# bcgsc/RNA-Bloom

Measured on AMD Instinct MI355X. Metric: k-mers/sec hashed+inserted into Bloom dBG (k=25, 50M 150bp reads), higher is better.
Workload: dtype u64

## Files before the change

rna-bloom_amd/csrc/rb_batch.hip:

```cpp
#include <math.h>
#include <stdlib.h>
#include <string.h>

#include <algorithm>
#include <vector>

#include "rb_internal.hpp"
#include "rb_kernels.hpp"

using namespace rb;

namespace {

constexpr int TPB = 256;
inline unsigned blocks_for(int64_t n, int tpb = TPB) { return (unsigned)((n + tpb - 1) / tpb); }

template <bool PIECE>
__global__ void k_encode_ascii_t(const uint8_t *__restrict__ seq, const uint8_t *__restrict__ qual,
                                 const int64_t *__restrict__ off, const uint32_t *__restrict__ woff,
                                 int64_t n_reads, int64_t n_words, int min_q,
                                 uint64_t *__restrict__ codes, uint32_t *__restrict__ valid,
                                 uint32_t *__restrict__ word_read, uint32_t *__restrict__ rnz,
                                 int64_t r_first, int64_t seq_base) {
    int64_t w = (int64_t)blockIdx.x * blockDim.x + threadIdx.x;
// ... 580 lines not shown
                      uint64_t *__restrict__ keys, uint32_t *__restrict__ vals, const uint32_t *__restrict__ keepmask,
                      const ulonglong2 *__restrict__ wstate) {
    constexpr uint32_t SLAB = RB_EMIT_SLAB, BW = RB_SPARSE_WORDS;
    __shared__ uint64_t s_key[SLAB + SLAB / 32 + 1];
    __shared__ uint32_t s_val[SLAB + SLAB / 32 + 1];
    __shared__ uint64_t s_tf[25], s_tr[25];
    __shared__ uint16_t s_list[BW];
    const uint32_t uk = (uint32_t)k, lane = threadIdx.x;
    const int64_t blk0 = (int64_t)blockIdx.x * BW;
    const int64_t blk_end = (blk0 + BW < nw) ? blk0 + BW : nw;
    const uint32_t O0 = chunk_off[blk0], O1 = chunk_off[blk_end];
    if (O0 == O1) return;
    if (threadIdx.x < 25) {
        const uint32_t o = threadIdx.x / 5u, in = threadIdx.x % 5u;
        const uint64_t so = o ? seed_of(o - 1u) : 0ull, si = in ? seed_of(in - 1u) : 0ull;
        const uint64_t sco = o ? seed_of(4u - o) : 0ull, sci = in ? seed_of(4u - in) : 0ull;
        s_tf[threadIdx.x] = rotl(so, uk) ^ si;
        s_tr[threadIdx.x] = rotr(sco, 1) ^ rotl(sci, uk - 1u);
    }
    uint32_t n_list = 0;
    for (uint32_t q = 0; q < BW; q += 64u) {
        const int64_t i = blk0 + q + lane;
        const bool ne = i < blk_end && chunk_off[i + 1] != chunk_off[i];
        const unsigned long long m = __builtin_amdgcn_ballot_w64(ne);
        if (ne) s_list[n_list + __builtin_amdgcn_mbcnt_hi((uint32_t)(m >> 32), __builtin_amdgcn_mbcnt_lo((uint32_t)m, 0u))] = (uint16_t)(q + lane);
        n_list += (uint32_t)__popcll(m);
    }
    __syncthreads();
    for (uint32_t e0 = 0; e0 < n_list; e0 += 64u) {
        const uint32_t e_last = (e0 + 64u < n_list) ? e0 + 63u : n_list - 1u;
        const uint32_t R0 = chunk_off[blk0 + s_list[e0]] - O0, R1 = chunk_off[blk0 + s_list[e_last] + 1] - O0;
        uint64_t ins = 0, outs = 0, f = 0, rv = 0;
        uint32_t inv = 0, outv = 0, j = 0, out = 0, rel = 0, b0 = 0, keep = 0;
        if (e0 + lane < n_list) {
            const int64_t i = blk0 + s_list[e0 + lane];
            const int64_t w = w0 + i;
            const uint32_t r = word_read[w], wr = woff[r], L = len[r];
            const uint32_t c = (uint32_t)(w - wr);
            b0 = c * 32u;
            keep = keepmask[i];
            const uint32_t nwords = (L + 31u) >> 5;
            const uint64_t cur = codes[w];
            const uint32_t curv = valid[w];
            const uint32_t pl = c ? (uint32_t)(codes[w - 1] >> 62) : 0u, plv = c ? (valid[w - 1] >> 31) : 0u;
            outs = (cur << 2) | pl;  outv = (curv << 1) | plv;
            const uint32_t q = (uk - 1u) >> 5, sh = (uk - 1u) & 31u;
            const uint64_t lo = q ? ((c + q < nwords) ? codes[w + q] : 0ull) : cur, hi = (c + q + 1u < nwords) ? codes[w + q + 1u] : 0ull;
            const uint32_t lov = q ? ((c + q < nwords) ? valid[w + q] : 0u) : curv, hiv = (c + q + 1u < nwords) ? valid[w + q + 1u] : 0u;
            ins = sh ? ((lo >> (2u * sh)) | (hi << (64u - 2u * sh))) : lo;
            inv = sh ? ((lov >> sh) | (hiv << (32u - sh))) : lov;
            const ulonglong2 st = wstate[i];
            f = st.x; rv = st.y;
            out = chunk_off[i] - O0;
            rel = (r - first_read) << pos_bits;
        }
        for (uint32_t slab0 = R0; slab0 < R1; slab0 += SLAB) {
            const uint32_t slab1 = (slab0 + SLAB < R1) ? slab0 + SLAB : R1;
            while (j < 32u && (keep >> j) != 0u && out < slab1) {
                const uint32_t in5 = (inv & 1u) ? ((uint32_t)ins & 3u) + 1u : 0u;
                const uint32_t out5 = (outv & 1u) ? ((uint32_t)outs & 3u) + 1u : 0u;
                ins >>= 2; inv >>= 1; outs >>= 2; outv >>= 1;
                const uint32_t t = out5 * 5u + in5;
                if (MODE != 2) f = rotl(f, 1) ^ s_tf[t];
                if (MODE != 0) rv = rotr(rv, 1) ^ s_tr[t];
                if ((keep >> j) & 1u) {
                    const uint32_t o = out - slab0, q = o + (o >> 5);
                    s_key[q] = (MODE == 0) ? f : (MODE == 2) ? rv : canonical(f, rv);
                    s_val[q] = rel | (b0 + j);
                    ++out;
                }
                ++j;
            }
            __syncthreads();
            for (uint32_t x = threadIdx.x; x < slab1 - slab0; x += 64u) {
                const uint32_t q = x + (x >> 5);
                keys[O0 + slab0 + x] = s_key[q];
                vals[O0 + slab0 + x] = s_val[q];
            }
            __syncthreads();
        }
    }
}

struct alignas(16) Emit4 { uint64_t f, r; };
struct Emit4Tab {
    Emit4 e[256];
    static constexpr uint64_t rot(uint64_t v, uint32_t s) { return s ? (v << s) | (v >> (64u - s)) : v; }
    constexpr Emit4Tab() : e{} {
        constexpr uint64_t sd[4] = {0x3c8bfbb395c60474ull, 0x3193c18562a02b4cull, 0x20323ed082572324ull, 0x295549f54be24456ull};
        for (uint32_t b = 0; b < 256u; ++b)
            for (uint32_t t = 0; t < 4u; ++t) {
                const uint32_t c = (b >> (2u * t)) & 3u;
                e[b].f ^= rot(sd[c], 3u - t);
                e[b].r ^= rot(sd[3u - c], t);
            }
    }
};
__device__ const Emit4Tab d_emit4 = Emit4Tab();
__device__ __forceinline__ uint64_t rotl4(uint64_t v) {
    const uint32_t lo = (uint32_t)v, hi = (uint32_t)(v >> 32);
    return ((uint64_t)__builtin_amdgcn_alignbit(hi, lo, 28) << 32) | __builtin_amdgcn_alignbit(lo, hi, 28);
}
__device__ __forceinline__ uint64_t rotr4(uint64_t v) {
    const uint32_t lo = (uint32_t)v, hi = (uint32_t)(v >> 32);
    return ((uint64_t)__builtin_amdgcn_alignbit(lo, hi, 4) << 32) | __builtin_amdgcn_alignbit(hi, lo, 4);
}
__device__ __forceinline__ uint32_t nth_set_bit(uint32_t m, uint32_t rank) {
    uint32_t pos = 0;
#pragma unroll
    for (uint32_t h = 16u; h; h >>= 1) {
        const uint32_t c = (uint32_t)__popc(m & ((1u << h) - 1u));
        const bool up = rank >= c;
        rank = up ? rank - c : rank; pos = up ? pos + h : pos; m = up ? m >> h : m;
    }
    return pos;
}
constexpr int EMIT_TPB = 256;
template <int MODE>
__global__ void __launch_bounds__(EMIT_TPB)
k_hash_windows_direct(const uint64_t *__restrict__ codes, const uint32_t *__restrict__ word_read, const uint32_t *__restrict__ woff,
                      int64_t w0, int64_t nw, int64_t n_words, int k, const uint32_t *__restrict__ chunk_off, uint32_t first_read,
                      uint32_t pos_bits, uint64_t *__restrict__ keys, uint32_t *__restrict__ vals, const uint32_t *__restrict__ keepmask) {
    constexpr uint32_t BW = RB_SPARSE_WORDS;
    static_assert((BW & (BW - 1u)) == 0u, "the offset search halves a power of two");
    __shared__ Emit4 s_t4[256];
    __shared__ uint64_t s_code[BW + 1];
    __shared__ uint32_t s_off[BW + 1], s_keep[BW], s_base[BW];
    const uint32_t tid = threadIdx.x;
    const int64_t blk0 = (int64_t)blockIdx.x * BW;
    const uint32_t nwb = (uint32_t)((blk0 + BW < nw ? blk0 + BW : nw) - blk0);
    const uint32_t O0 = chunk_off[blk0], n = chunk_off[blk0 + nwb] - O0;
    if (n == 0u) return;
    for (uint32_t i = tid; i < 256u; i += EMIT_TPB) s_t4[i] = d_emit4.e[i];
    for (uint32_t i = tid; i <= BW; i += EMIT_TPB) {
        uint32_t o = 0xFFFFFFFFu;
        uint64_t c = 0;
        if (i <= nwb) {
            const int64_t w = w0 + blk0 + i;
            o = chunk_off[blk0 + i] - O0;
            if (w < n_words) c = codes[w];
            if (i < nwb && chunk_off[blk0 + i + 1] - O0 != o) {
                const uint32_t r = word_read[w];
                s_keep[i] = keepmask[blk0 + i];
                s_base[i] = ((r - first_read) << pos_bits) + ((uint32_t)w - woff[r]) * 32u;
            }
        }
        s_off[i] = o; s_code[i] = c;
    }
    __syncthreads();
    const uint32_t uk = (uint32_t)k, nq = (uk + 3u) >> 2, pad = 4u * nq - uk;
    const uint32_t mask_lo = uk >= 16u ? 0xFFFFFFFFu : (1u << (2u * uk)) - 1u;
    const uint32_t mask_hi = uk >= 32u ? 0xFFFFFFFFu : uk <= 16u ? 0u : (1u << (2u * uk - 32u)) - 1u;
    uint64_t fx = 0, rx = 0;
    for (uint32_t t = 4u - pad; t < 4u; ++t) { fx ^= rotl(seed_of(0u), 3u - t); rx ^= rotl(seed_of(3u), t); }
    const uint32_t sf = (uk - 4u * nq) & 63u, sr = 4u * (nq - 1u);
    for (uint32_t x = tid; x < n; x += EMIT_TPB) {
        uint32_t pos = 0;
#pragma unroll
        for (uint32_t step = BW >> 1; step; step >>= 1) pos = (s_off[pos + step] <= x) ? pos + step : pos;
        const uint32_t j = nth_set_bit(s_keep[pos], x - s_off[pos]);
        const uint64_t c0 = s_code[pos], c1 = s_code[pos + 1u];
        uint32_t a = (uint32_t)c0, b = (uint32_t)(c0 >> 32), c = (uint32_t)c1;
        if (j & 16u) { a = b; b = c; c = (uint32_t)(c1 >> 32); }
        const uint32_t sh = (2u * j) & 31u;
        const uint32_t wlo = __builtin_amdgcn_alignbit(b, a, sh) & mask_lo, whi = __builtin_amdgcn_alignbit(c, b, sh) & mask_hi;
        uint64_t f = 0, r = 0;
#pragma unroll
        for (uint32_t q = 0; q < 8u; ++q) {
            if (q >= nq) break;
            const Emit4 e = s_t4[((q < 4u ? wlo : whi) >> (8u * (q & 3u))) & 0xFFu];
            if (MODE != 2) f = rotl4(f) ^ e.f;
            if (MODE != 0) r = rotr4(r) ^ e.r;
        }
        if (MODE != 2) f = rotl_var(f ^ fx, sf);
        if (MODE != 0) r = rotl_var(r ^ rx, sr);
        keys[O0 + x] = (MODE == 0) ? f : (MODE == 2) ? r : canonical(f, r);
        vals[O0 + x] = s_base[pos] + j;
    }
}
__global__ void k_emit_compare(const uint64_t *__restrict__ ka, const uint32_t *__restrict__ va, const uint64_t *__restrict__ kb,
                               const uint32_t *__restrict__ vb, uint32_t n, uint32_t *__restrict__ res) {
    const uint32_t i = blockIdx.x * blockDim.x + threadIdx.x;
    if (i < n && (ka[i] != kb[i] || va[i] != vb[i])) { atomicAdd(&res[0], 1u); atomicMin(&res[1], i); }
}

constexpr int RB_READ_WORDS = 10;

template <int MODE, bool MPF>
__global__ void __launch_bounds__(64)
// ... 1063 lines not shown
```

rna-bloom_amd/csrc/rb_device.hpp:

```cpp
#pragma once
#include <hip/hip_runtime.h>
#include <stdint.h>

namespace rb {

__device__ __forceinline__ uint64_t seed_of(uint32_t code) {
    uint64_t s = 0x3c8bfbb395c60474ull;
    s = (code == 1) ? 0x3193c18562a02b4cull : s;
    s = (code == 2) ? 0x20323ed082572324ull : s;
    s = (code == 3) ? 0x295549f54be24456ull : s;
    return s;
}
__device__ __forceinline__ uint64_t rotl1(uint64_t v) {
    const uint32_t lo = (uint32_t)v, hi = (uint32_t)(v >> 32);
    return ((uint64_t)__builtin_amdgcn_alignbit(hi, lo, 31) << 32) | __builtin_amdgcn_alignbit(lo, hi, 31);
}
__device__ __forceinline__ uint64_t rotr1(uint64_t v) {
    const uint32_t lo = (uint32_t)v, hi = (uint32_t)(v >> 32);
    return ((uint64_t)__builtin_amdgcn_alignbit(lo, hi, 1) << 32) | __builtin_amdgcn_alignbit(hi, lo, 1);
}
__device__ __forceinline__ uint64_t rotl(uint64_t v, uint32_t s) {
    if (__builtin_constant_p(s) && s == 1u) return rotl1(v);
    s &= 63u;
    return (v << s) | (v >> ((64u - s) & 63u));
// ... 249 lines not shown
        const uint32_t ha_b = mpf_slot_b(ha);
        if (!__hip_atomic_load(&b[ha_b], __ATOMIC_RELAXED, __HIP_MEMORY_SCOPE_AGENT)) {
            __hip_atomic_store(&b[ha_b], (mpf_tag_b(ha) << 3) | (ea & 7ull), __ATOMIC_RELAXED, __HIP_MEMORY_SCOPE_AGENT);
            __hip_atomic_store(&b[sa], na, __ATOMIC_RELAXED, __HIP_MEMORY_SCOPE_AGENT);
            return true;
        }
        const uint64_t hb = (((eb >> 6) << 3 | (uint64_t)(sb >> 1)) << 3) | ((eb >> 3) & 7ull);
        const uint32_t hb_a = mpf_slot_a(hb);
        if (!__hip_atomic_load(&b[hb_a], __ATOMIC_RELAXED, __HIP_MEMORY_SCOPE_AGENT)) {
            __hip_atomic_store(&b[hb_a], (mpf_tag_a(hb) << 3) | (eb & 7ull), __ATOMIC_RELAXED, __HIP_MEMORY_SCOPE_AGENT);
            __hip_atomic_store(&b[sb], nb, __ATOMIC_RELAXED, __HIP_MEMORY_SCOPE_AGENT);
            return true;
        }
    }
    {
        const uint64_t ha = ((ea >> 3) << 3) | (uint64_t)(sa >> 1);
        const uint32_t ha_b = mpf_slot_b(ha);
        const unsigned long long ec = __hip_atomic_load(&b[ha_b], __ATOMIC_RELAXED, __HIP_MEMORY_SCOPE_AGENT);
        if (ec && ha_b != sb) {
            const uint64_t hc = (((ec >> 6) << 3 | (uint64_t)(ha_b >> 1)) << 3) | ((ec >> 3) & 7ull);
            const uint32_t hc_a = mpf_slot_a(hc);
            if (hc_a != sa && !__hip_atomic_load(&b[hc_a], __ATOMIC_RELAXED, __HIP_MEMORY_SCOPE_AGENT)) {
                __hip_atomic_store(&b[hc_a], (mpf_tag_a(hc) << 3) | (ec & 7ull), __ATOMIC_RELAXED, __HIP_MEMORY_SCOPE_AGENT);
                __hip_atomic_store(&b[ha_b], (mpf_tag_b(ha) << 3) | (ea & 7ull), __ATOMIC_RELAXED, __HIP_MEMORY_SCOPE_AGENT);
                __hip_atomic_store(&b[sa], na, __ATOMIC_RELAXED, __HIP_MEMORY_SCOPE_AGENT);
                return true;
            }
        }
        const uint64_t hb = (((eb >> 6) << 3 | (uint64_t)(sb >> 1)) << 3) | ((eb >> 3) & 7ull);
        const uint32_t hb_a = mpf_slot_a(hb);
        const unsigned long long ed = __hip_atomic_load(&b[hb_a], __ATOMIC_RELAXED, __HIP_MEMORY_SCOPE_AGENT);
        if (ed && hb_a != sa) {
            const uint64_t hd = ((ed >> 3) << 3) | (uint64_t)(hb_a >> 1);
            const uint32_t hd_b = mpf_slot_b(hd);
            if (hd_b != sb && !__hip_atomic_load(&b[hd_b], __ATOMIC_RELAXED, __HIP_MEMORY_SCOPE_AGENT)) {
                __hip_atomic_store(&b[hd_b], (mpf_tag_b(hd) << 3) | (ed & 7ull), __ATOMIC_RELAXED, __HIP_MEMORY_SCOPE_AGENT);
                __hip_atomic_store(&b[hb_a], (mpf_tag_a(hb) << 3) | (eb & 7ull), __ATOMIC_RELAXED, __HIP_MEMORY_SCOPE_AGENT);
                __hip_atomic_store(&b[sb], nb, __ATOMIC_RELAXED, __HIP_MEMORY_SCOPE_AGENT);
                return true;
            }
        }
    }
    const bool pick_b = mpf_rank((uint32_t)(eb & 7ull)) < mpf_rank((uint32_t)(ea & 7ull));
    if (mpf_rank((uint32_t)((pick_b ? eb : ea) & 7ull)) < rv) { __hip_atomic_store(&b[pick_b ? sb : sa], pick_b ? nb : na, __ATOMIC_RELAXED, __HIP_MEMORY_SCOPE_AGENT); return true; }
    return false;
}
__device__ __forceinline__ uint32_t mpf_match(const unsigned long long *bkt, uint32_t stride, uint64_t h0) {
    const unsigned long long ea = bkt[mpf_slot_a(h0) * stride], eb = bkt[mpf_slot_b(h0) * stride];
    uint32_t s = 0;
    if (ea && (ea >> 3) == mpf_tag_a(h0)) { const uint32_t v = (uint32_t)(ea & 7ull); s = v ? v : RB_MPF_TOP_EXP; }
    if (eb && (eb >> 3) == mpf_tag_b(h0)) { const uint32_t v = (uint32_t)(eb & 7ull), r = v ? v : RB_MPF_TOP_EXP; s = r > s ? r : s; }
    return s;
}

__device__ __forceinline__ uint32_t mpf_match_entries(unsigned long long ea, unsigned long long eb, uint64_t h0);
__device__ __forceinline__ uint32_t mpf_match_flat(const unsigned long long *bkt, uint32_t stride, uint64_t h0) {
    return mpf_match_entries(bkt[mpf_slot_a(h0) * stride], bkt[mpf_slot_b(h0) * stride], h0);
}
__device__ __forceinline__ uint32_t mpf_match_entries(unsigned long long ea, unsigned long long eb, uint64_t h0) {
    const uint32_t va = (uint32_t)(ea & 7ull), vb = (uint32_t)(eb & 7ull);
    const uint32_t ha = (uint32_t)(((ea ^ (mpf_tag_a(h0) << 3)) < 8ull) & (ea != 0ull));
    const uint32_t hb = (uint32_t)(((eb ^ (mpf_tag_b(h0) << 3)) < 8ull) & (eb != 0ull));
    const uint32_t ra = ha ? (va ? va : RB_MPF_TOP_EXP) : 0u;
    const uint32_t rb = hb ? (vb ? vb : RB_MPF_TOP_EXP) : 0u;
    return ra > rb ? ra : rb;
}

__host__ __device__ __forceinline__ uint32_t draw_strength(uint32_t rnd31) {
    const uint32_t r = rnd31 | 0x8000u;
#if defined(__HIP_DEVICE_COMPILE__)
    return (uint32_t)__ffs((int)r) - 1u;
#else
    return (uint32_t)__builtin_ctz(r);
#endif
}

__device__ __forceinline__ bool bit_test(const uint32_t *bits, uint64_t i) {
    return (bits[i >> 5] >> (uint32_t)(i & 31u)) & 1u;
}
__device__ __forceinline__ void bit_set(uint32_t *bits, uint64_t i) {
    uint32_t m = 1u << (uint32_t)(i & 31u);
    if (!(bits[i >> 5] & m)) atomicOr(&bits[i >> 5], m);
}
__device__ __forceinline__ bool bits_lookup(const uint32_t *bits, const Mod &mod, int num_hash, uint64_t kmul, uint64_t h0) {
    for (int j = 0; j < num_hash; ++j)
        if (!bit_test(bits, index_of(multi_hash(h0, (uint32_t)j, kmul), mod))) return false;
    return true;
}

}
```

rna-bloom_amd/csrc/rb_graph.hip:

```cpp
#include <math.h>
#include <stdarg.h>
#include <stdlib.h>
#include <string.h>
#include <time.h>

#include <algorithm>
#include <new>
#include <vector>

#include <functional>
#include <string>
#include <thread>

#include <fcntl.h>
#include <unistd.h>
#include <zlib.h>

#include "rb_pipeline.hpp"

using namespace rb;

namespace rb {
static thread_local char g_err[768] = "";
const char *last_error_text() { return g_err; }
// ... 773 lines not shown
            fR = rotl(fR, 1) ^ seed_of(cr); rR ^= rotl(seed_of(3u - cr), q);
        }
        for (;;) {
            uint64_t P;
            if (MODE == 0) P = combine(fL, fR);
            else if (MODE == 2) P = combine(rR, rL);
            else P = smin(combine(fL, fR), combine(rR, rL));
            if (OUT) {
                for (int j = 0; j < num_hash; ++j)
                    out_idx[((size_t)chunk_off[i] + cnt) * (size_t)num_hash + j] = index_of(multi_hash(P, (uint32_t)j, kmul), mod);
            } else {
                for (int j = 0; j < num_hash; ++j) bit_set(bits, index_of(multi_hash(P, (uint32_t)j, kmul), mod));
            }
            ++cnt;
            if (p == plast) break;
            const uint32_t ol = code_at(p), il = code_at(p + uk), orr = code_at(p + ud), ir = code_at(p + ud + uk);
            fL = rotl(fL, 1) ^ rotl(seed_of(ol), uk) ^ seed_of(il);
            rL = rotr(rL, 1) ^ rotr(seed_of(3u - ol), 1) ^ rotl(seed_of(3u - il), uk - 1u);
            fR = rotl(fR, 1) ^ rotl(seed_of(orr), uk) ^ seed_of(ir);
            rR = rotr(rR, 1) ^ rotr(seed_of(3u - orr), 1) ^ rotl(seed_of(3u - ir), uk - 1u);
            ++p;
        }
        p = plast + 1u;
    }
    if (cnt && n_pairs) atomicAdd(n_pairs, (unsigned long long)cnt);
}


#ifdef RB_DIAG_PAIRS
__global__ void k_pairs_insert_runtime_branch(const uint64_t *__restrict__ codes, const uint32_t *__restrict__ valid,
                               const uint32_t *__restrict__ word_read, const uint32_t *__restrict__ woff,
                               const uint32_t *__restrict__ len, int64_t w0, int64_t nw, int k, int dist,
                               uint32_t *bits, Mod mod, int num_hash, uint64_t kmul,
                               unsigned long long *__restrict__ n_pairs,
                               const uint32_t *__restrict__ chunk_off, uint64_t *__restrict__ out_idx,
                               uint32_t wpr_uniform) {
    int64_t t = (int64_t)blockIdx.x * blockDim.x + threadIdx.x;
    if (t >= nw) return;
    int64_t i = t;
    if (wpr_uniform) { const int64_t nreads = nw / wpr_uniform; i = (t % nreads) * wpr_uniform + t / nreads; }
    const int64_t w = w0 + i;
    const uint32_t r = word_read[w], wr = woff[r], L = len[r];
    const uint32_t b0 = (uint32_t)(w - wr) * 32u;
    const uint32_t uk = (uint32_t)k, ud = (uint32_t)dist, span = uk + ud;
    if ((uint64_t)b0 + span > L) return;
    const uint32_t pe = (b0 + 32u < L - span + 1u) ? b0 + 32u : L - span + 1u;
    const uint64_t *cw = codes + wr;
    const uint32_t *vw = valid + wr;
    auto code_at = [&](uint32_t b) { return (uint32_t)(cw[b >> 5] >> (2u * (b & 31u))) & 3u; };
    uint32_t cnt = 0, p = b0;
    while (p < pe) {
        const uint32_t nz = next_unusable(vw, p, L);
        if (nz < p + span) { p = nz + 1u; continue; }
        const uint32_t plast = (pe - 1u < nz - span) ? pe - 1u : nz - span;
        uint64_t fL = 0, rL = 0, fR = 0, rR = 0;
        for (uint32_t q = 0; q < uk; ++q) {
            const uint32_t cl = code_at(p + q), cr = code_at(p + ud + q);
            fL = rotl(fL, 1) ^ seed_of(cl); rL ^= rotl(seed_of(3u - cl), q);
            fR = rotl(fR, 1) ^ seed_of(cr); rR ^= rotl(seed_of(3u - cr), q);
        }
        for (;;) {
            const uint64_t P = smin(combine(fL, fR), combine(rR, rL));
            if (out_idx) {
                for (int j = 0; j < num_hash; ++j)
                    out_idx[((size_t)chunk_off[i] + cnt) * (size_t)num_hash + j] = index_of(multi_hash(P, (uint32_t)j, kmul), mod);
            } else {
                for (int j = 0; j < num_hash; ++j) bit_set(bits, index_of(multi_hash(P, (uint32_t)j, kmul), mod));
            }
            ++cnt;
            if (p == plast) break;
            const uint32_t ol = code_at(p), il = code_at(p + uk), orr = code_at(p + ud), ir = code_at(p + ud + uk);
            fL = rotl(fL, 1) ^ rotl(seed_of(ol), uk) ^ seed_of(il);
            rL = rotr(rL, 1) ^ rotr(seed_of(3u - ol), 1) ^ rotl(seed_of(3u - il), uk - 1u);
            fR = rotl(fR, 1) ^ rotl(seed_of(orr), uk) ^ seed_of(ir);
            rR = rotr(rR, 1) ^ rotr(seed_of(3u - orr), 1) ^ rotl(seed_of(3u - ir), uk - 1u);
            ++p;
        }
        p = plast + 1u;
    }
    if (cnt && n_pairs) atomicAdd(n_pairs, (unsigned long long)cnt);
}
#endif

template <int MODE, int PAIR_WORDS, int VAR>
__global__ void __launch_bounds__(64)
k_pairs_reads(const uint64_t *__restrict__ codes, const uint32_t *__restrict__ valid, const uint32_t *__restrict__ woff,
              const uint32_t *__restrict__ len, int64_t r0, int64_t nr, int64_t w0, int k, int dist, uint32_t *bits, Mod mod,
              int num_hash, uint64_t kmul, unsigned long long *__restrict__ n_pairs, const uint32_t *__restrict__ chunk_off,
              uint64_t *__restrict__ out_idx, uint32_t min_len, const uint32_t *__restrict__ present, Mod present_mod, int present_h,
              PairSeen seen) {
    __shared__ uint64_t s_tf[25], s_tr[25];
    __shared__ unsigned long long s_img[VAR == 1 ? 16 * 64 : 1];
    const uint32_t uk = (uint32_t)k, ud = (uint32_t)dist, span = uk + ud;
    const uint32_t um = uk < 16u ? uk : 16u;
    if (threadIdx.x < 25) {
        const uint32_t o = threadIdx.x / 5u, in = threadIdx.x % 5u;
        const uint64_t so = o ? seed_of(o - 1u) : 0ull, si = in ? seed_of(in - 1u) : 0ull;
        const uint64_t sco = o ? seed_of(4u - o) : 0ull, sci = in ? seed_of(4u - in) : 0ull;
        s_tf[threadIdx.x] = rotl(so, uk) ^ si;
        s_tr[threadIdx.x] = rotr(sco, 1) ^ rotl(sci, uk - 1u);
    }
    __syncthreads();
    const int64_t t = (int64_t)blockIdx.x * 64 + threadIdx.x;
    uint32_t cnt = 0;
    if (t < nr) {
        const int64_t r = r0 + t;
        const uint32_t wr = woff[r], L = len[r];
        if (L >= span && L >= min_len) {
            const uint32_t nwords = (L + 31u) >> 5;
            uint64_t carr[PAIR_WORDS];
            uint32_t varr[PAIR_WORDS];
#pragma unroll
            for (int q = 0; q < PAIR_WORDS; ++q) {
                carr[q] = 0; varr[q] = 0;
                if ((uint32_t)q < nwords) { carr[q] = codes[wr + q]; varr[q] = valid[wr + q]; }
            }
            uint32_t lb = 0;
#pragma unroll
            for (int q = 0; q < PAIR_WORDS; ++q) {
                if (32u * (uint32_t)q < ud) {
                    const uint32_t hi = ud - 32u * (uint32_t)q;
                    const uint32_t m = ~varr[q] & (hi >= 32u ? 0xFFFFFFFFu : ((1u << hi) - 1u));
                    if (m) lb = 32u * (uint32_t)q + 32u - (uint32_t)__clz((int)m);
                }
            }
            auto word_c = [&](uint32_t wi) { uint64_t v = 0;
#pragma unroll
                for (int q = 0; q < PAIR_WORDS; ++q) v = ((uint32_t)q == wi) ? carr[q] : v;
                return v; };
            auto word_v = [&](uint32_t wi) { uint32_t v = 0;
#pragma unroll
                for (int q = 0; q < PAIR_WORDS; ++q) v = ((uint32_t)q == wi) ? varr[q] : v;
                return v; };
            uint64_t cR = word_c(ud >> 5) >> (2u * (ud & 31u)), cL = carr[0];
            uint32_t vR = word_v(ud >> 5) >> (ud & 31u), vL = varr[0];
            uint64_t fR = 0, rR = 0, fL = 0, rL = 0, hcR = 0, hcR2 = 0, hcL = 0, hcL2 = 0, hvR = 0, hvL = 0;
            const uint32_t sh_v = uk - 1u, sh_c = 2u * ((uk - 1u) & 31u);
            const bool far = uk > 32u;
            const uint32_t nsteps = L - ud;
            const int64_t wrel = (int64_t)wr - w0;
            uint32_t obase = 0, ocnt = 0, oword = 0xFFFFFFFFu;
            uint32_t mF = 0, mR = 0;
            const uint32_t mmask = um >= 16u ? 0xFFFFFFFFu : ((1u << (2u * um)) - 1u), mtop = 2u * (um - 1u);
            uint32_t akey = 0, apos1 = 0, xnew = 0, curb = 0xFFFFFFFFu;
            uint32_t dbg_miss = 0, dbg_fetch = 0;
#pragma nounroll
            for (uint32_t j = 0; j < nsteps; ++j) {
                const uint32_t e = ud + j;
                if (j && (e & 31u) == 0u) { cR = word_c(e >> 5); vR = word_v(e >> 5); }
                if (j && (j & 31u) == 0u) { cL = word_c(j >> 5); vL = word_v(j >> 5); }
                const uint32_t codeR = (uint32_t)cR & 3u, okR = vR & 1u, codeL = (uint32_t)cL & 3u, okL = vL & 1u;
                cR >>= 2; vR >>= 1; cL >>= 2; vL >>= 1;
                {
                    const uint32_t in5 = okR ? codeR + 1u : 0u;
                    const uint32_t out5 = ((uint32_t)(hvR >> sh_v) & 1u) ? ((uint32_t)((far ? hcR2 : hcR) >> sh_c) & 3u) + 1u : 0u;
                    const uint32_t tt = out5 * 5u + in5;
                    fR = rotl(fR, 1) ^ s_tf[tt]; rR = rotr(rR, 1) ^ s_tr[tt];
                    hcR2 = (hcR2 << 2) | (hcR >> 62); hcR = (hcR << 2) | codeR; hvR = (hvR << 1) | okR;
                }
                {
                    const uint32_t in5 = okL ? codeL + 1u : 0u;
                    const uint32_t out5 = ((uint32_t)(hvL >> sh_v) & 1u) ? ((uint32_t)((far ? hcL2 : hcL) >> sh_c) & 3u) + 1u : 0u;
                    const uint32_t tt = out5 * 5u + in5;
                    fL = rotl(fL, 1) ^ s_tf[tt]; rL = rotr(rL, 1) ^ s_tr[tt];
                    if (VAR == 1) {
                        mF = ((mF << 2) | codeL) & mmask;
                        mR = (mR >> 2) | ((3u - codeL) << mtop);
                        uint32_t x = (mF < mR ? mF : mR) * 0x9E3779B1u;
                        x ^= x >> 15;
                        xnew = x >> 4;
                        if ((x & seen.amask) == 0u && j + 1u >= um) { akey = xnew; apos1 = j + 2u - um; }
                    }
                    hcL2 = (hcL2 << 2) | (hcL >> 62); hcL = (hcL << 2) | codeL; hvL = (hvL << 1) | okL;
                }
                lb = okR ? lb : e + 1u;
                if (j + 1u >= uk) {
                    const uint32_t p = j + 1u - uk;
                    bool ok = lb <= p;
                    if (ok && present) {
                        const uint64_t hl = (MODE == 0) ? fL : (MODE == 2) ? rL : smin(fL, rL);
                        const uint64_t hr = (MODE == 0) ? fR : (MODE == 2) ? rR : smin(fR, rR);
                        ok = bits_lookup(present, present_mod, present_h, kmul, hl) && bits_lookup(present, present_mod, present_h, kmul, hr);
                    }
                    if (ok) {
                        uint64_t P;
                        if (MODE == 0) P = combine(fL, fR);
                        else if (MODE == 2) P = combine(rR, rL);
                        else P = smin(combine(fL, fR), combine(rR, rL));
                        if (VAR == 2) {
                            if ((p >> 5) != oword) { oword = p >> 5; obase = chunk_off[wrel + (int64_t)oword]; ocnt = 0; }
                            for (int h = 0; h < num_hash; ++h)
                                out_idx[((size_t)obase + ocnt) * (size_t)num_hash + h] = index_of(multi_hash(P, (uint32_t)h, kmul), mod);
                            ++ocnt;
                        } else if (VAR == 1) {
                            const uint32_t bk = (apos1 > p ? akey : xnew) & seen.mask;
                            if (bk != curb) {
                                curb = bk; ++dbg_fetch;
                                const uint4 *src = reinterpret_cast<const uint4 *>(seen.tab + ((size_t)bk << 4));
                                uint4 v[8];
#pragma unroll
                                for (int q = 0; q < 8; ++q) v[q] = src[q];
#pragma unroll
                                for (int q = 0; q < 8; ++q) {
                                    s_img[(2 * q) * 64 + threadIdx.x] = (unsigned long long)v[q].x | ((unsigned long long)v[q].y << 32);
                                    s_img[(2 * q + 1) * 64 + threadIdx.x] = (unsigned long long)v[q].z | ((unsigned long long)v[q].w << 32);
                                }
                            }
                            const uint32_t sa = (uint32_t)P & 15u, sb0 = ((uint32_t)P >> 4) & 15u, sb = sb0 == sa ? (sa ^ 1u) : sb0;
                            const unsigned long long ea = s_img[sa * 64u + threadIdx.x], eb = s_img[sb * 64u + threadIdx.x];
                            if (P == 0ull || (ea != P && eb != P)) {
                                ++dbg_miss;
                                for (int h = 0; h < num_hash; ++h) bit_set(bits, index_of(multi_hash(P, (uint32_t)h, kmul), mod));
                                if (P != 0ull) {
                                    const uint32_t sl = ea == 0ull ? sa : (eb == 0ull ? sb : sa);
                                    s_img[sl * 64u + threadIdx.x] = P;
                                    seen.tab[((size_t)bk << 4) + sl] = P;
                                }
                            }
                        } else {
                            for (int h = 0; h < num_hash; ++h) bit_set(bits, index_of(multi_hash(P, (uint32_t)h, kmul), mod));
                        }
                        ++cnt;
                    }
                }
            }
            if (VAR == 1 && seen.dbg) { atomicAdd(seen.dbg, (unsigned long long)dbg_miss); atomicAdd(seen.dbg + 1, (unsigned long long)dbg_fetch); }
        }
    }
    if (n_pairs) {
        unsigned long long c = cnt;
        for (int o = 32; o > 0; o >>= 1) c += __shfl_down(c, o, 64);
        if (threadIdx.x == 0 && c) atomicAdd(n_pairs, c);
    }
}

}

void rb::launch_pairs_reads(rb_graph *g, const rb_batch *b, int64_t w0, int64_t nw, int mode_hash, const BitFilter &f, int dist,
                               uint32_t min_len, bool if_present, const uint32_t *chunk_off, uint64_t *out_idx, unsigned long long *pc,
                               hipStream_t st) {
    RB_REQUIRE(g->k <= 64 && b->max_len <= 1024u, "paired k-mers: k <= 64 and reads of at most 1024 bases only on this path");
    const auto &wo = b->h_woff;
    const int64_t r0 = std::lower_bound(wo.begin(), wo.end(), (uint32_t)w0) - wo.begin();
    const int64_t r1 = std::lower_bound(wo.begin(), wo.end(), (uint32_t)(w0 + nw)) - wo.begin();
    RB_REQUIRE(r0 < (int64_t)wo.size() && wo[(size_t)r0] == (uint32_t)w0 && r1 < (int64_t)wo.size() && wo[(size_t)r1] == (uint32_t)(w0 + nw),
               "launch_pairs: word range does not start and end at read boundaries");
    if (r1 <= r0) return;
    dim3 gr(blocks_for(r1 - r0, 64)), th(64);
    const uint32_t *present = if_present ? g->dbg.bits : nullptr;
    const bool use_seen = f.seen && !out_idx && !present;
    static const uint32_t anchor_bits = getenv("RB_PAIR_SEEN_ANCHOR") ? (uint32_t)std::max(0, std::min(4, atoi(getenv("RB_PAIR_SEEN_ANCHOR")))) : 2u;
    const PairSeen seen{use_seen ? f.seen : nullptr, use_seen ? (1u << f.seen_log2b) - 1u : 0u, (1u << anchor_bits) - 1u,
                        (use_seen && pc == g->pairs_ctr.as<unsigned long long>() && getenv("RB_DEBUG")) ? pc + 1 : nullptr};
#define RB_LAUNCH_PR3(M, NW, V)                                                                                          \
    hipLaunchKernelGGL((k_pairs_reads<M, NW, V>), gr, th, 0, st, b->codes, b->valid, b->woff, b->len, r0, r1 - r0, w0, g->k, \
                       dist, f.bits, f.mod, f.num_hash, kmul_of(g->k), pc, chunk_off, out_idx, min_len, present, g->dbg.mod, g->dbg.num_hash, seen)
#define RB_LAUNCH_PR(M, NW) do { if (out_idx) RB_LAUNCH_PR3(M, NW, 2); else if (use_seen) RB_LAUNCH_PR3(M, NW, 1); else RB_LAUNCH_PR3(M, NW, 0); } while (0)
    if (b->max_len <= 384u) { if (mode_hash == 0) RB_LAUNCH_PR(0, 12); else if (mode_hash == 2) RB_LAUNCH_PR(2, 12); else RB_LAUNCH_PR(1, 12); }
    else { if (mode_hash == 0) RB_LAUNCH_PR(0, 32); else if (mode_hash == 2) RB_LAUNCH_PR(2, 32); else RB_LAUNCH_PR(1, 32); }
#undef RB_LAUNCH_PR
#undef RB_LAUNCH_PR3
}

void rb::launch_pairs(rb_graph *g, const rb_batch *b, int64_t w0, int64_t nw, int mode_hash, const uint32_t *chunk_off,
                      uint64_t *out_idx, unsigned long long *pc, hipStream_t st, const BitFilter *into) {
    if (!st) st = g->stream;
    if (nw <= 0) return;
    const BitFilter &rpk = into ? *into : g->rpk;
    const bool general = g->k > 64 || b->max_len > 384u || (getenv("RB_PAIRS_GENERAL") && atoi(getenv("RB_PAIRS_GENERAL")));
    if (!general) {
        launch_pairs_reads(g, b, w0, nw, mode_hash, rpk, g->read_d, 0u, false, chunk_off, out_idx, pc, st);
        return;
    }
    dim3 gr(blocks_for(nw)), th(TPB);
#ifdef RB_DIAG_PAIRS
    if (getenv("RB_PAIRS_VARIANT") && atoi(getenv("RB_PAIRS_VARIANT")) == 9 && mode_hash == 1) {
        hipLaunchKernelGGL(k_pairs_insert_runtime_branch, gr, th, 0, st, b->codes, b->valid, b->word_read, b->woff, b->len, w0, nw, g->k, g->read_d,
                           rpk.bits, rpk.mod, rpk.num_hash, kmul_of(g->k), pc, chunk_off, out_idx,
                           (b->wpr_uniform && nw % b->wpr_uniform == 0) ? b->wpr_uniform : 0u);
        return;
    }
#endif
#define RB_LAUNCH_PAIRS(M)                                                                                          \
    if (out_idx) RB_LAUNCH_PAIRS2(M, true); else RB_LAUNCH_PAIRS2(M, false)
#define RB_LAUNCH_PAIRS2(M, O)                                                                                      \
    hipLaunchKernelGGL((k_pairs_insert<M, O>), gr, th, 0, st, b->codes, b->valid, b->word_read, b->woff, b->len, w0, nw, \
                       g->k, g->read_d, rpk.bits, rpk.mod, rpk.num_hash, kmul_of(g->k), pc, chunk_off, out_idx, \
                       (b->wpr_uniform && nw % b->wpr_uniform == 0) ? b->wpr_uniform : 0u)
    if (mode_hash == 0) { RB_LAUNCH_PAIRS(0); } else if (mode_hash == 2) { RB_LAUNCH_PAIRS(2); } else { RB_LAUNCH_PAIRS(1); }
#undef RB_LAUNCH_PAIRS
#undef RB_LAUNCH_PAIRS2
}

static bool sweep_wanted(const rb_graph *g) {
    if (g->shard || !g->dbg.bits || g->dbg.lo != 0 || g->dbg.hi != g->dbg.size) return false;
    if (const char *e = getenv("RB_SWEEP")) return atoi(e) != 0;
    return g->dbg.nbytes >= ((int64_t)1 << 31);
}
void rb::group_enqueue(rb_graph *g, int slot, size_t N, uint64_t ordinal0, uint32_t pos_bits, hipStream_t st, DevBuf &temp,
                       DevBuf &ctrbuf, int flags) {
    rb_graph::GroupSlot &S = g->slots[slot];
    S.N = N; S.D = 0; S.flags = flags; S.live = (uint32_t)N;
    ctrbuf.reserve(DEVCTR_BYTES);
    uint32_t *ctr = ctrbuf.as<uint32_t>();
    RB_HIP(hipMemsetAsync(ctr, 0, DEVCTR_BYTES, st));
    if (N == 0) return;
    const int group_bits = 64 - g->sort_begin_bit;
    const int bucket_target = g->shard ? (getenv("RB_SHARD_GROUP_TARGET") ? atoi(getenv("RB_SHARD_GROUP_TARGET")) : 3072) : 0;
    S.bucket_target = bucket_target;
    temp.reserve(group_temp_bytes(N, group_bits, bucket_target, flags));
    S.keys1.reserve(N * 8); S.valsT.reserve(N * 4); S.vals1.reserve(N * 4); S.tz.reserve(N + 16);
    S.uniq.reserve(N * 8); S.counts.reserve((N + 1) * 4); S.starts.reserve((N + 1) * 4);
    GrIdx gidx{Mod{1, 0, 0}, 0, 0};
    bool want_idx = true;
    if (const char *e = getenv("RB_GROUP_IDX")) want_idx = atoi(e) != 0;
    if (want_idx) {
        if (g->cbf && g->cbf_size > 0) gidx = GrIdx{g->cbf_mod, (uint64_t)g->cbf_lo, (uint64_t)(g->cbf_hi - g->cbf_lo)};
        else if (g->dbg.bits && g->dbg.size > 0) gidx = GrIdx{g->dbg.mod, (uint64_t)g->dbg.lo, (uint64_t)(g->dbg.hi - g->dbg.lo)};
    }
    GroupExport ex;
    S.sweep_T = 0; S.n_main = 0;
    if (want_idx && sweep_wanted(g)) {
        const GrIdx didx{g->dbg.mod, 0, (uint64_t)g->dbg.size};
        const bool same = gidx.span == didx.span && gidx.lo == 0 && gidx.mod.d == didx.mod.d;
        if (!same) gidx = didx;
        S.sweep_T = group_index_buckets(N, group_bits, bucket_target, flags, gidx);
        if (S.sweep_T) {
            S.brun.reserve(((size_t)4 << S.sweep_T) + 16); S.bnr.reserve(((size_t)4 << S.sweep_T) + 16);
            ex = GroupExport{S.brun.as<uint32_t>(), S.bnr.as<uint32_t>(), ctr + 9};
        }
    }
    uint64_t *kin = g->group_in_keys ? g->group_in_keys : g->keys0.as<uint64_t>();
    uint32_t *vin = g->group_in_vals ? g->group_in_vals : g->vals0.as<uint32_t>();
    g->group_in_keys = nullptr; g->group_in_vals = nullptr;
    group_records_device(kin, vin, S.keys1.as<uint64_t>(), S.valsT.as<uint32_t>(), N, group_bits,
                         g->p.rng_seed, ordinal0, pos_bits, temp.p, temp.cap, S.vals1.as<uint32_t>(), S.tz.as<uint8_t>(), S.uniq.as<uint64_t>(),
                         S.counts.as<uint32_t>(), S.starts.as<uint32_t>(), ctr + 8, st, g, bucket_target, flags, gidx, ex);
}
uint32_t rb::group_finish(rb_graph *g, int slot, hipStream_t st, DevBuf &temp, DevBuf &ctrbuf, hipStream_t scan_stream) {
    rb_graph::GroupSlot &S = g->slots[slot];
    if (S.N == 0) { RB_HIP(hipStreamSynchronize(st)); return 0; }
    uint32_t D = 0;
    RB_HIP(hipMemcpyAsync(&D, ctrbuf.as<uint32_t>() + 8, 4, hipMemcpyDeviceToHost, st));
    if (S.sweep_T) RB_HIP(hipMemcpyAsync(&S.n_main, ctrbuf.as<uint32_t>() + 9, 4, hipMemcpyDeviceToHost, st));
// ... 656 lines not shown
```

Baseline: 43.96 billion.

## Seed paired k-mer hashes directly via 2-base table and unroll two-hash inserts

For k<=32, the paired-read kernel now builds the initial left and right ntHash windows in one pass using a 16-entry two-base lookup table kept in shared memory, then corrects for invalid bases. Outgoing bases are taken from the original code words instead of shifting history registers. This removes the k-1 warm-up roll steps and the per-step history maintenance. It also adds a bits_add helper that, when there are two hashes, issues both bit-word loads before either conditional atomic so their latencies overlap. The costs are more code complexity, a new template variant, and extra register pressure.

```diff
diff --git a/rna-bloom_amd/csrc/rb_batch.hip b/rna-bloom_amd/csrc/rb_batch.hip
--- a/rna-bloom_amd/csrc/rb_batch.hip
+++ b/rna-bloom_amd/csrc/rb_batch.hip
@@ -686,29 +686,6 @@
     }
 }
 
-struct alignas(16) Emit4 { uint64_t f, r; };
-struct Emit4Tab {
-    Emit4 e[256];
-    static constexpr uint64_t rot(uint64_t v, uint32_t s) { return s ? (v << s) | (v >> (64u - s)) : v; }
-    constexpr Emit4Tab() : e{} {
-        constexpr uint64_t sd[4] = {0x3c8bfbb395c60474ull, 0x3193c18562a02b4cull, 0x20323ed082572324ull, 0x295549f54be24456ull};
-        for (uint32_t b = 0; b < 256u; ++b)
-            for (uint32_t t = 0; t < 4u; ++t) {
-                const uint32_t c = (b >> (2u * t)) & 3u;
-                e[b].f ^= rot(sd[c], 3u - t);
-                e[b].r ^= rot(sd[3u - c], t);
-            }
-    }
-};
-__device__ const Emit4Tab d_emit4 = Emit4Tab();
-__device__ __forceinline__ uint64_t rotl4(uint64_t v) {
-    const uint32_t lo = (uint32_t)v, hi = (uint32_t)(v >> 32);
-    return ((uint64_t)__builtin_amdgcn_alignbit(hi, lo, 28) << 32) | __builtin_amdgcn_alignbit(lo, hi, 28);
-}
-__device__ __forceinline__ uint64_t rotr4(uint64_t v) {
-    const uint32_t lo = (uint32_t)v, hi = (uint32_t)(v >> 32);
-    return ((uint64_t)__builtin_amdgcn_alignbit(lo, hi, 4) << 32) | __builtin_amdgcn_alignbit(hi, lo, 4);
-}
 __device__ __forceinline__ uint32_t nth_set_bit(uint32_t m, uint32_t rank) {
     uint32_t pos = 0;
 #pragma unroll
diff --git a/rna-bloom_amd/csrc/rb_device.hpp b/rna-bloom_amd/csrc/rb_device.hpp
--- a/rna-bloom_amd/csrc/rb_device.hpp
+++ b/rna-bloom_amd/csrc/rb_device.hpp
@@ -355,10 +355,57 @@
     uint32_t m = 1u << (uint32_t)(i & 31u);
     if (!(bits[i >> 5] & m)) atomicOr(&bits[i >> 5], m);
 }
+__device__ __forceinline__ void bits_add(uint32_t *bits, const Mod &mod, int num_hash, uint64_t kmul, uint64_t h0) {
+    if (num_hash == 2) {
+        const uint64_t i0 = index_of(multi_hash(h0, 0u, kmul), mod), i1 = index_of(multi_hash(h0, 1u, kmul), mod);
+        const uint32_t m0 = 1u << (uint32_t)(i0 & 31u), m1 = 1u << (uint32_t)(i1 & 31u);
+        const uint32_t w0 = bits[i0 >> 5], w1 = bits[i1 >> 5];
+        if (!(w0 & m0)) atomicOr(&bits[i0 >> 5], m0);
+        if (!(w1 & m1)) atomicOr(&bits[i1 >> 5], m1);
+        return;
+    }
+    for (int j = 0; j < num_hash; ++j) bit_set(bits, index_of(multi_hash(h0, (uint32_t)j, kmul), mod));
+}
 __device__ __forceinline__ bool bits_lookup(const uint32_t *bits, const Mod &mod, int num_hash, uint64_t kmul, uint64_t h0) {
     for (int j = 0; j < num_hash; ++j)
         if (!bit_test(bits, index_of(multi_hash(h0, (uint32_t)j, kmul), mod))) return false;
     return true;
 }
 
-}
+struct alignas(16) Emit4 { uint64_t f, r; };
+template <uint32_t B>
+struct EmitTab {
+    Emit4 e[1u << (2u * B)];
+    static constexpr uint64_t rot(uint64_t v, uint32_t s) { return s ? (v << s) | (v >> (64u - s)) : v; }
+    constexpr EmitTab() : e{} {
+        constexpr uint64_t sd[4] = {0x3c8bfbb395c60474ull, 0x3193c18562a02b4cull, 0x20323ed082572324ull, 0x295549f54be24456ull};
+        for (uint32_t b = 0; b < (1u << (2u * B)); ++b)
+            for (uint32_t t = 0; t < B; ++t) {
+                const uint32_t c = (b >> (2u * t)) & 3u;
+                e[b].f ^= rot(sd[c], B - 1u - t);
+                e[b].r ^= rot(sd[3u - c], t);
+            }
+    }
+};
+using Emit4Tab = EmitTab<4>;
+using Emit2Tab = EmitTab<2>;
+static __device__ const Emit4Tab d_emit4 = Emit4Tab();
+static __device__ const Emit2Tab d_emit2 = Emit2Tab();
+__device__ __forceinline__ uint64_t rotl4(uint64_t v) {
+    const uint32_t lo = (uint32_t)v, hi = (uint32_t)(v >> 32);
+    return ((uint64_t)__builtin_amdgcn_alignbit(hi, lo, 28) << 32) | __builtin_amdgcn_alignbit(lo, hi, 28);
+}
+__device__ __forceinline__ uint64_t rotr4(uint64_t v) {
+    const uint32_t lo = (uint32_t)v, hi = (uint32_t)(v >> 32);
+    return ((uint64_t)__builtin_amdgcn_alignbit(lo, hi, 4) << 32) | __builtin_amdgcn_alignbit(hi, lo, 4);
+}
+__device__ __forceinline__ uint64_t rotl2(uint64_t v) {
+    const uint32_t lo = (uint32_t)v, hi = (uint32_t)(v >> 32);
+    return ((uint64_t)__builtin_amdgcn_alignbit(hi, lo, 30) << 32) | __builtin_amdgcn_alignbit(lo, hi, 30);
+}
+__device__ __forceinline__ uint64_t rotr2(uint64_t v) {
+    const uint32_t lo = (uint32_t)v, hi = (uint32_t)(v >> 32);
+    return ((uint64_t)__builtin_amdgcn_alignbit(lo, hi, 2) << 32) | __builtin_amdgcn_alignbit(hi, lo, 2);
+}
+
+}
diff --git a/rna-bloom_amd/csrc/rb_graph.hip b/rna-bloom_amd/csrc/rb_graph.hip
--- a/rna-bloom_amd/csrc/rb_graph.hip
+++ b/rna-bloom_amd/csrc/rb_graph.hip
@@ -879,7 +879,7 @@
 }
 #endif
 
-template <int MODE, int PAIR_WORDS, int VAR>
+template <int MODE, int PAIR_WORDS, int VAR, bool DIRECT>
 __global__ void __launch_bounds__(64)
 k_pairs_reads(const uint64_t *__restrict__ codes, const uint32_t *__restrict__ valid, const uint32_t *__restrict__ woff,
               const uint32_t *__restrict__ len, int64_t r0, int64_t nr, int64_t w0, int k, int dist, uint32_t *bits, Mod mod,
@@ -888,8 +888,10 @@
               PairSeen seen) {
     __shared__ uint64_t s_tf[25], s_tr[25];
     __shared__ unsigned long long s_img[VAR == 1 ? 16 * 64 : 1];
+    __shared__ Emit4 s_t2[DIRECT ? 16 : 1];
     const uint32_t uk = (uint32_t)k, ud = (uint32_t)dist, span = uk + ud;
     const uint32_t um = uk < 16u ? uk : 16u;
+    if (DIRECT && threadIdx.x < 16) s_t2[threadIdx.x] = d_emit2.e[threadIdx.x];
     if (threadIdx.x < 25) {
         const uint32_t o = threadIdx.x / 5u, in = threadIdx.x % 5u;
         const uint64_t so = o ? seed_of(o - 1u) : 0ull, si = in ? seed_of(in - 1u) : 0ull;
@@ -912,11 +914,12 @@
                 carr[q] = 0; varr[q] = 0;
                 if ((uint32_t)q < nwords) { carr[q] = codes[wr + q]; varr[q] = valid[wr + q]; }
             }
+            const uint32_t lbe = DIRECT ? span : ud;
             uint32_t lb = 0;
 #pragma unroll
             for (int q = 0; q < PAIR_WORDS; ++q) {
-                if (32u * (uint32_t)q < ud) {
-                    const uint32_t hi = ud - 32u * (uint32_t)q;
+                if (32u * (uint32_t)q < lbe) {
+                    const uint32_t hi = lbe - 32u * (uint32_t)q;
                     const uint32_t m = ~varr[q] & (hi >= 32u ? 0xFFFFFFFFu : ((1u << hi) - 1u));
                     if (m) lb = 32u * (uint32_t)q + 32u - (uint32_t)__clz((int)m);
                 }
@@ -941,37 +944,89 @@
             const uint32_t mmask = um >= 16u ? 0xFFFFFFFFu : ((1u << (2u * um)) - 1u), mtop = 2u * (um - 1u);
             uint32_t akey = 0, apos1 = 0, xnew = 0, curb = 0xFFFFFFFFu;
             uint32_t dbg_miss = 0, dbg_fetch = 0;
+            auto mmer_step = [&](uint32_t codeL, uint32_t j) {
+                mF = ((mF << 2) | codeL) & mmask;
+                mR = (mR >> 2) | ((3u - codeL) << mtop);
+                uint32_t x = (mF < mR ? mF : mR) * 0x9E3779B1u;
+                x ^= x >> 15;
+                xnew = x >> 4;
+                if ((x & seen.amask) == 0u && j + 1u >= um) { akey = xnew; apos1 = j + 2u - um; }
+            };
+            uint64_t oR = 0, oL = 0;
+            uint32_t uR = 0, uL = 0;
+            if (DIRECT) {
+                const uint32_t wi = ud >> 5, sv = ud & 31u, sc = 2u * sv, e0 = span;
+                const uint64_t wa = word_c(wi), wb = word_c(wi + 1u);
+                const uint32_t va = word_v(wi), vb = word_v(wi + 1u);
+                oL = carr[0]; uL = varr[0]; oR = wa >> sc; uR = va >> sv;
+                const uint64_t cmask = uk >= 32u ? ~0ull : ((1ull << (2u * uk)) - 1ull);
+                const uint32_t kmask = uk >= 32u ? 0xFFFFFFFFu : ((1u << uk) - 1u);
+                const uint64_t wl = oL & cmask, wr = (sc ? (oR | (wb << (64u - sc))) : oR) & cmask;
+                const uint32_t zl = ~uL & kmask, zr = ~(sv ? (uR | (vb << (32u - sv))) : uR) & kmask;
+                const uint32_t nq = (uk + 1u) >> 1, pad = 2u * nq - uk;
+                uint64_t xl = wl, xr = wr;
+                for (uint32_t q = 0; q < nq; ++q) {
+                    const Emit4 el = s_t2[(uint32_t)xl & 15u], er = s_t2[(uint32_t)xr & 15u];
+                    xl >>= 4; xr >>= 4;
+                    fL = rotl2(fL) ^ el.f; rL = rotr2(rL) ^ el.r;
+                    fR = rotl2(fR) ^ er.f; rR = rotr2(rR) ^ er.r;
+                }
+                const uint64_t fx = pad ? seed_of(0u) : 0ull, rx = pad ? rotl(seed_of(3u), 1) : 0ull;
+                const uint32_t sf = (64u - pad) & 63u, sr = 2u * (nq - 1u);
+                fL = rotl_var(fL ^ fx, sf); rL = rotl_var(rL ^ rx, sr);
+                fR = rotl_var(fR ^ fx, sf); rR = rotl_var(rR ^ rx, sr);
+                auto drop = [&](uint32_t z, uint64_t w, uint64_t &f, uint64_t &r) {
+                    while (z) {
+                        const uint32_t i = (uint32_t)__ffs((int)z) - 1u;
+                        z &= z - 1u;
+                        const uint32_t c = (((i & 16u) ? (uint32_t)(w >> 32) : (uint32_t)w) >> (2u * (i & 15u))) & 3u;
+                        f ^= rotl_var(seed_of(c), uk - 1u - i); r ^= rotl_var(seed_of(3u - c), i);
+                    }
+                };
+                drop(zl, wl, fL, rL);
+                drop(zr, wr, fR, rR);
+                cL = uk >= 32u ? carr[1] : carr[0] >> (2u * uk); vL = uk >= 32u ? varr[1] : varr[0] >> uk;
+                cR = ((e0 >> 5) == wi ? wa : wb) >> (2u * (e0 & 31u)); vR = ((e0 >> 5) == wi ? va : vb) >> (e0 & 31u);
+                if (VAR == 1) {
+                    uint64_t x64 = carr[0];
+                    for (uint32_t j = 0; j < uk; ++j) { mmer_step((uint32_t)x64 & 3u, j); x64 >>= 2; }
+                }
+            }
 #pragma nounroll
-            for (uint32_t j = 0; j < nsteps; ++j) {
+            for (uint32_t j = DIRECT ? uk - 1u : 0u; j < nsteps; ++j) {
                 const uint32_t e = ud + j;
-                if (j && (e & 31u) == 0u) { cR = word_c(e >> 5); vR = word_v(e >> 5); }
-                if (j && (j & 31u) == 0u) { cL = word_c(j >> 5); vL = word_v(j >> 5); }
-                const uint32_t codeR = (uint32_t)cR & 3u, okR = vR & 1u, codeL = (uint32_t)cL & 3u, okL = vL & 1u;
-                cR >>= 2; vR >>= 1; cL >>= 2; vL >>= 1;
-                {
-                    const uint32_t in5 = okR ? codeR + 1u : 0u;
-                    const uint32_t out5 = ((uint32_t)(hvR >> sh_v) & 1u) ? ((uint32_t)((far ? hcR2 : hcR) >> sh_c) & 3u) + 1u : 0u;
-                    const uint32_t tt = out5 * 5u + in5;
-                    fR = rotl(fR, 1) ^ s_tf[tt]; rR = rotr(rR, 1) ^ s_tr[tt];
-                    hcR2 = (hcR2 << 2) | (hcR >> 62); hcR = (hcR << 2) | codeR; hvR = (hvR << 1) | okR;
+                if (!DIRECT || j >= uk) {
+                    if (j && (e & 31u) == 0u) { cR = word_c(e >> 5); vR = word_v(e >> 5); }
+                    if (j && (j & 31u) == 0u) { cL = word_c(j >> 5); vL = word_v(j >> 5); }
+                    const uint32_t codeR = (uint32_t)cR & 3u, okR = vR & 1u, codeL = (uint32_t)cL & 3u, okL = vL & 1u;
+                    cR >>= 2; vR >>= 1; cL >>= 2; vL >>= 1;
+                    if (DIRECT) {
+                        const uint32_t gl = j - uk, gr = e - uk;
+                        if (gl && (gr & 31u) == 0u) { oR = word_c(gr >> 5); uR = word_v(gr >> 5); }
+                        if (gl && (gl & 31u) == 0u) { oL = word_c(gl >> 5); uL = word_v(gl >> 5); }
+                    }
+                    {
+                        const uint32_t in5 = okR ? codeR + 1u : 0u;
+                        uint32_t out5;
+                        if (DIRECT) { out5 = (uR & 1u) ? ((uint32_t)oR & 3u) + 1u : 0u; oR >>= 2; uR >>= 1; }
+                        else out5 = ((uint32_t)(hvR >> sh_v) & 1u) ? ((uint32_t)((far ? hcR2 : hcR) >> sh_c) & 3u) + 1u : 0u;
+                        const uint32_t tt = out5 * 5u + in5;
+                        fR = rotl(fR, 1) ^ s_tf[tt]; rR = rotr(rR, 1) ^ s_tr[tt];
+                        if (!DIRECT) { hcR2 = (hcR2 << 2) | (hcR >> 62); hcR = (hcR << 2) | codeR; hvR = (hvR << 1) | okR; }
+                    }
+                    {
+                        const uint32_t in5 = okL ? codeL + 1u : 0u;
+                        uint32_t out5;
+                        if (DIRECT) { out5 = (uL & 1u) ? ((uint32_t)oL & 3u) + 1u : 0u; oL >>= 2; uL >>= 1; }
+                        else out5 = ((uint32_t)(hvL >> sh_v) & 1u) ? ((uint32_t)((far ? hcL2 : hcL) >> sh_c) & 3u) + 1u : 0u;
+                        const uint32_t tt = out5 * 5u + in5;
+                        fL = rotl(fL, 1) ^ s_tf[tt]; rL = rotr(rL, 1) ^ s_tr[tt];
+                        if (VAR == 1) mmer_step(codeL, j);
+                        if (!DIRECT) { hcL2 = (hcL2 << 2) | (hcL >> 62); hcL = (hcL << 2) | codeL; hvL = (hvL << 1) | okL; }
+                    }
+                    lb = okR ? lb : e + 1u;
                 }
-                {
-                    const uint32_t in5 = okL ? codeL + 1u : 0u;
-                    const uint32_t out5 = ((uint32_t)(hvL >> sh_v) & 1u) ? ((uint32_t)((far ? hcL2 : hcL) >> sh_c) & 3u) + 1u : 0u;
-                    const uint32_t tt = out5 * 5u + in5;
-                    fL = rotl(fL, 1) ^ s_tf[tt]; rL = rotr(rL, 1) ^ s_tr[tt];
-                    if (VAR == 1) {
-                        mF = ((mF << 2) | codeL) & mmask;
-                        mR = (mR >> 2) | ((3u - codeL) << mtop);
-                        uint32_t x = (mF < mR ? mF : mR) * 0x9E3779B1u;
-                        x ^= x >> 15;
-                        xnew = x >> 4;
-                        if ((x & seen.amask) == 0u && j + 1u >= um) { akey = xnew; apos1 = j + 2u - um; }
-                    }
-                    hcL2 = (hcL2 << 2) | (hcL >> 62); hcL = (hcL << 2) | codeL; hvL = (hvL << 1) | okL;
-                }
-                lb = okR ? lb : e + 1u;
-                if (j + 1u >= uk) {
+                if (DIRECT || j + 1u >= uk) {
                     const uint32_t p = j + 1u - uk;
                     bool ok = lb <= p;
                     if (ok && present) {
@@ -1007,7 +1062,7 @@
                             const unsigned long long ea = s_img[sa * 64u + threadIdx.x], eb = s_img[sb * 64u + threadIdx.x];
                             if (P == 0ull || (ea != P && eb != P)) {
                                 ++dbg_miss;
-                                for (int h = 0; h < num_hash; ++h) bit_set(bits, index_of(multi_hash(P, (uint32_t)h, kmul), mod));
+                                bits_add(bits, mod, num_hash, kmul, P);
                                 if (P != 0ull) {
                                     const uint32_t sl = ea == 0ull ? sa : (eb == 0ull ? sb : sa);
                                     s_img[sl * 64u + threadIdx.x] = P;
@@ -1015,7 +1070,7 @@
                                 }
                             }
                         } else {
-                            for (int h = 0; h < num_hash; ++h) bit_set(bits, index_of(multi_hash(P, (uint32_t)h, kmul), mod));
+                            bits_add(bits, mod, num_hash, kmul, P);
                         }
                         ++cnt;
                     }
@@ -1049,14 +1104,17 @@
     static const uint32_t anchor_bits = getenv("RB_PAIR_SEEN_ANCHOR") ? (uint32_t)std::max(0, std::min(4, atoi(getenv("RB_PAIR_SEEN_ANCHOR")))) : 2u;
     const PairSeen seen{use_seen ? f.seen : nullptr, use_seen ? (1u << f.seen_log2b) - 1u : 0u, (1u << anchor_bits) - 1u,
                         (use_seen && pc == g->pairs_ctr.as<unsigned long long>() && getenv("RB_DEBUG")) ? pc + 1 : nullptr};
-#define RB_LAUNCH_PR3(M, NW, V)                                                                                          \
-    hipLaunchKernelGGL((k_pairs_reads<M, NW, V>), gr, th, 0, st, b->codes, b->valid, b->woff, b->len, r0, r1 - r0, w0, g->k, \
+    const bool direct = g->k <= 32 && !(getenv("RB_PAIRS_DIRECT") && atoi(getenv("RB_PAIRS_DIRECT")) == 0);
+#define RB_LAUNCH_PR3(M, NW, V) do { if (direct) RB_LAUNCH_PR4(M, NW, V, true); else RB_LAUNCH_PR4(M, NW, V, false); } while (0)
+#define RB_LAUNCH_PR4(M, NW, V, D)                                                                                       \
+    hipLaunchKernelGGL((k_pairs_reads<M, NW, V, D>), gr, th, 0, st, b->codes, b->valid, b->woff, b->len, r0, r1 - r0, w0, g->k, \
                        dist, f.bits, f.mod, f.num_hash, kmul_of(g->k), pc, chunk_off, out_idx, min_len, present, g->dbg.mod, g->dbg.num_hash, seen)
 #define RB_LAUNCH_PR(M, NW) do { if (out_idx) RB_LAUNCH_PR3(M, NW, 2); else if (use_seen) RB_LAUNCH_PR3(M, NW, 1); else RB_LAUNCH_PR3(M, NW, 0); } while (0)
     if (b->max_len <= 384u) { if (mode_hash == 0) RB_LAUNCH_PR(0, 12); else if (mode_hash == 2) RB_LAUNCH_PR(2, 12); else RB_LAUNCH_PR(1, 12); }
     else { if (mode_hash == 0) RB_LAUNCH_PR(0, 32); else if (mode_hash == 2) RB_LAUNCH_PR(2, 32); else RB_LAUNCH_PR(1, 32); }
 #undef RB_LAUNCH_PR
 #undef RB_LAUNCH_PR3
+#undef RB_LAUNCH_PR4
 }
 
 void rb::launch_pairs(rb_graph *g, const rb_batch *b, int64_t w0, int64_t nw, int mode_hash, const uint32_t *chunk_off,
```

Result: no change. 44.07 billion, median of 6 (+0.2%).
